# ADVRHumanoids/CentroidalPlanner

Hardware: AMD Instinct MI355X
Metric: NLP eval_g+eval_jac_g throughput (rows/sec) at batch*contacts; HBM GB/s vs peak (higher is better)
Workload: dtype f64; 1 GPU; 4-contact Ground env, batch=1,048,576 (north-star target); contacts=4, environment=ground, batch_per_gpu=1048576, batch_total=1048576, outputs=g + jac (IFOPT CSR values), per-shard residual norms, parallelism=instance-sharded x1, launch=hip-graph, 10 steps per replay

## Files before the change

centroidalplanner_amd/_abi.py:

```python
from __future__ import annotations

import ctypes
import os
from ctypes import POINTER, c_char_p, c_double, c_int32, c_int64, c_size_t, c_uint8, c_void_p

MAX_CONTACTS = 32
ABI_VERSION = 1

ENV_NONE = 0
ENV_GROUND = 1
ENV_SUPERQUADRIC = 2
ENV_MIXED = 3

OK = 0
ERR_INVALID_ARGUMENT = 1
ERR_OUT_OF_RANGE = 2
ERR_RUNTIME = 3
ERR_HIP = 4
ERR_UNSUPPORTED = 5

INF = 1.0e20

EVAL_JAC_FOLDED = 1
EVAL_SOA = 2
# ... 105 lines not shown
    _fields_ = [
        ("d_wrench", c_void_p),
        ("d_com_ref", c_void_p),
        ("d_p_ref", c_void_p),
        ("d_F_ref", c_void_p),
    ]


class DerivativeReport(ctypes.Structure):

    _fields_ = [
        ("n_checked", c_int64),
        ("n_flagged", c_int64),
        ("max_rel_error", c_double),
        ("worst_instance", c_int64),
        ("worst_row", c_int32),
        ("worst_col", c_int32),
        ("worst_exact", c_double),
        ("worst_approx", c_double),
    ]


HESSIAN_EXACT = 0
HESSIAN_LIMITED_MEMORY = 1
HESSIAN_FD = 2
HESSIAN_ANALYTIC = 3

TERM_SCALED = 0
TERM_IPOPT = 1
SOLVE_DIVERGING = 5
SOLVE_TIME_LIMIT = 6

_DESC_P = POINTER(ProblemDesc)
_DP = POINTER(c_double)
_IP = POINTER(c_int32)
SIGNATURES = {
    "cpl_abi_version": (c_int32, []),
    "cpl_desc_sizeof": (c_size_t, []),
    "cpl_last_error": (c_char_p, []),
    "cpl_status_string": (c_char_p, [c_int32]),
    "cpl_desc_init": (c_int32, [_DESC_P, c_int32, c_int32, c_double]),
    "cpl_desc_set_contact_names": (c_int32, [_DESC_P, POINTER(c_char_p), c_int32]),
    "cpl_desc_set_mu": (c_int32, [_DESC_P, c_double]),
    "cpl_desc_set_superquadric": (c_int32, [_DESC_P, _DP, _DP, _DP]),
    "cpl_desc_set_bounds": (c_int32, [_DESC_P, c_int32, c_int32, _DP, _DP]),
    "cpl_dims": (c_int32, [_DESC_P, _IP, _IP, _IP]),
    "cpl_structure": (c_int32, [_DESC_P, _IP, _IP, _IP]),
    "cpl_bounds": (c_int32, [_DESC_P, _DP, _DP, _DP, _DP]),
    "cpl_eval_batch": (
        c_int32,
        [_DESC_P, c_int64, c_void_p, c_void_p, c_void_p, c_void_p, c_void_p, c_void_p, c_void_p, c_void_p],
    ),
    "cpl_set_tuning": (c_int32, [c_int32, c_int32, c_int32, c_int32, c_int32]),
    "cpl_residual_norms": (c_int32, [_DESC_P, c_int64, c_void_p, c_void_p, c_void_p]),
    "cpl_eval_batch_norms": (
        c_int32,
        [_DESC_P, c_int64, c_void_p, c_void_p, c_void_p, c_void_p, c_void_p, c_void_p, c_void_p, c_void_p, c_void_p],
    ),
    "cpl_time_eval_batch": (
        c_int32,
        [_DESC_P, c_int64, c_void_p, c_void_p, c_void_p, c_void_p, c_void_p, c_void_p, c_void_p, c_void_p,
         c_void_p, c_int32, _DP],
    ),
    "cpl_eval_batch_ex": (
        c_int32,
        [_DESC_P, c_int64, c_void_p, c_void_p, c_void_p, c_void_p, c_void_p, c_void_p, c_void_p, c_void_p, c_int32,
         c_void_p],
    ),
    "cpl_instance_data_sizeof": (c_size_t, []),
    "cpl_eval_batch_inst": (
        c_int32,
        [_DESC_P, c_int64, c_void_p, c_void_p, c_void_p, POINTER(InstanceDataC), c_void_p, c_void_p, c_void_p, c_void_p,
         c_void_p, c_int32, c_void_p],
    ),
    "cpl_jac_fold_info": (c_int32, [_DESC_P, _IP, _IP, _IP, _IP, _DP]),
    "cpl_time_eval_batch_ex": (
        c_int32,
        [_DESC_P, c_int64, c_void_p, c_void_p, c_void_p, c_void_p, c_void_p, c_void_p, c_void_p, c_void_p,
         c_int32, c_void_p, c_int32, _DP],
    ),
    "cpl_eval_batch_host": (
        c_int32,
        [_DESC_P, c_int64, c_void_p, c_void_p, c_void_p, c_void_p, c_void_p, c_void_p, c_void_p, c_void_p, c_int32],
    ),
    "cpl_derivative_test": (
        c_int32,
        [_DESC_P, c_int64, c_void_p, c_void_p, c_void_p, c_double, c_double, c_void_p, POINTER(DerivativeReport),
         c_void_p],
    ),
    "cpl_kkt_workspace_doubles": (c_int64, [c_int32, c_int32]),
    "cpl_lagrangian_hessian": (c_int32, [_DESC_P, c_int64, c_void_p, c_void_p, c_void_p, c_void_p, c_int32, c_void_p,
                                         c_void_p]),
    "cpl_lagrangian_hessian_ex": (c_int32, [_DESC_P, c_int64, c_void_p, c_void_p, c_void_p, c_void_p, c_void_p, c_int32,
                                            c_void_p, c_void_p]),
    "cpl_eval_lagrangian_grad": (
        c_int32,
        [_DESC_P, c_int64, c_void_p, c_void_p, c_void_p, c_void_p, c_void_p, c_void_p, c_void_p, c_int32, c_void_p,
         c_void_p, c_void_p],
    ),
    "cpl_lagrangian_grad": (
        c_int32,
        [c_int64, c_int32, c_int32, c_int32, c_void_p, c_void_p, c_void_p, c_void_p, c_void_p, c_void_p, c_int32,
         c_void_p, c_void_p],
    ),
    "cpl_kkt_qd_solve": (c_int32, [c_int64, c_int32, c_int32] + [c_void_p] * 12),
    "cpl_kkt_solve": (
# ... 120 lines not shown
```

centroidalplanner_amd/csrc/cpl_kernels.hip:

```cpp
#include <hip/hip_runtime.h>

#include <cmath>
#include <cstdlib>
#include <cstring>
#include <map>
#include <mutex>
#include <string>
#include <tuple>
#include <vector>

#include "cpl_accept.hpp"
#include "cpl_engine.hpp"
#include "cpl_kkt_block.hpp"
#include "cpl_kkt_wave.hpp"
#include "cpl_layout.hpp"
#include "cpl_wave.hpp"
#include "cpl_status.hpp"

namespace cpl {

constexpr int TILE = 64;
constexpr int CHUNK = 16;
constexpr int SROW = CHUNK + 2;

struct KParams {
  int32_t N, n, m, nnz;
  int32_t env_kind;
  int32_t has_env;
  int32_t x_aligned16;
  int32_t pad0;
  int8_t map_order[CPL_MAX_CONTACTS];
  double mass_default;
  double gravity[3];
  double wrench[6];
  double mu;
  double ground_z;
  double C[3], R[3], P[3];
  double EJ[3];
  double Ka[3];
  double Kb[3];
  double Rm2[3];
  double Rp2[3];
  double Psq[3], Pm1[3], P2[3], P2m2[3], P2m3[3];
  double F_thr[CPL_MAX_CONTACTS];
  double W_com, com_ref[3];
  double W_p[CPL_MAX_CONTACTS], W_F[CPL_MAX_CONTACTS];
  double p_ref[CPL_MAX_CONTACTS][3], F_ref[CPL_MAX_CONTACTS][3];
  int32_t T, logT;
  int32_t S;
  int32_t cost_seg;
  int32_t offG, offJ, offD, offL, offI;
  int32_t LR;
  int32_t offX1, offMB, offTB;
  int32_t want_g, want_j, want_f, want_grad;
  int32_t want_norms;
  int32_t contact_rows;
  int32_t sq_ladder;
  int32_t grid_cap;
  int32_t want_lgrad, y_repeat;
  const int32_t* col_ptr;
  const int32_t* csc_k;
  const int32_t* csc_row;
  const double* ly;
  const uint8_t* lg_active;
  int32_t offC;
  int32_t fold, jbase, cstride;
  int32_t soa;
  int32_t jdirect;
  int32_t offA;
  int32_t offRB, offCS, offST;
  const double* sc_df;
  const double* sc_dc;
  const int32_t* sc_row;
  const uint8_t* gate;
};
static_assert(sizeof(KParams) < 4096, "kernel parameters must fit the kernarg segment");

constexpr int CPL_MAX_ROWS = 6 + 6 * CPL_MAX_CONTACTS;
enum { AX_C, AX_R, AX_P, AX_EJ, AX_KA, AX_KB, AX_RM2, AX_RP2, AX_PSQ, AX_PM1, AX_P2, AX_P2M2, AX_P2M3, AX_N };
struct CTab {
  int32_t map_order[CPL_MAX_CONTACTS];
  double F_thr[CPL_MAX_CONTACTS];
  double ax[AX_N][3];
  uint8_t cone[CPL_MAX_ROWS];
};
__shared__ CTab s_ct;

__device__ __forceinline__ void load_ctab(const KParams& K) {
  const int t = threadIdx.x;
  if (t < CPL_MAX_CONTACTS) {
    s_ct.map_order[t] = K.map_order[t];
    s_ct.F_thr[t] = K.F_thr[t];
  }
  if (t < 3 * AX_N) {
    const int f = t / 3, a = t - 3 * (t / 3);
    double v;
    switch (f) {
      case AX_C: v = K.C[a]; break;
      case AX_R: v = K.R[a]; break;
      case AX_P: v = K.P[a]; break;
      case AX_EJ: v = K.EJ[a]; break;
      case AX_KA: v = K.Ka[a]; break;
      case AX_KB: v = K.Kb[a]; break;
      case AX_RM2: v = K.Rm2[a]; break;
      case AX_RP2: v = K.Rp2[a]; break;
      case AX_PSQ: v = K.Psq[a]; break;
      case AX_PM1: v = K.Pm1[a]; break;
      case AX_P2: v = K.P2[a]; break;
      case AX_P2M2: v = K.P2m2[a]; break;
      default: v = K.P2m3[a]; break;
    }
    s_ct.ax[f][a] = v;
  }
  for (int r = t; r < K.m; r += blockDim.x)
    s_ct.cone[r] = r >= 6 && ((r - 6) % K.contact_rows) >= K.contact_rows - 2;
}

__device__ __forceinline__ double row_violation(double g, bool cone) {
  if (g != g) return INFINITY;
  if (cone) return g > 0.0 ? g : 0.0;
  return fabs(g);
}

struct NormAcc {
  double vmax = 0.0, vsum = 0.0;
  int r = 0, rstep = 0;
  __device__ void init(int tid, int nthreads, int m) {
// ... 1282 lines not shown
        for (int e = tid; e < valid * n; e += WG) {
          const int r = e / n;
          grad_out[rowb[r] * n + (e - r * n)] = Dt[e];
        }
    } else if (K.soa) {
      if (K.want_g) copy_out_soa<WG, NT>(g_out + b0, batch, Gt, m, valid, tid);
      if (K.want_j) copy_out_soa<WG, NT>(jac_out + b0, batch, Jt, nnz, valid, tid);
      if (K.want_grad) copy_out_soa<WG, NT>(grad_out + b0, batch, Dt, n, valid, tid);
    } else {
      if (K.want_g) copy_out<WG, NT>(g_out + b0 * m, Gt, valid * m, tid);
      if (K.want_j && !JD) copy_out<WG, NT>(jac_out + b0 * nnz, Jt, valid * nnz, tid);
      if (K.want_grad) copy_out<WG, NT>(grad_out + b0 * n, Dt, valid * n, tid);
    }
  }
}
using TileKernT = void (*)(const KParams, int64_t, const double*, const double*, const uint8_t*, const int32_t*,
                           const int32_t*, double*, double*, double*, double*, double*);


typedef __attribute__((address_space(3))) void lds_void_t;
typedef __attribute__((address_space(1))) void glb_void_t;


__device__ __forceinline__ void dma_tile(double* dst, const double* src, int count, int lane) {
  const int pieces = (count + 127) >> 7;
  for (int p = 0; p < pieces; ++p) {
    const int e = p * 128 + lane * 2;
    if (e + 1 < count) __builtin_amdgcn_global_load_lds((glb_void_t*)(src + e), (lds_void_t*)(dst + p * 128), 16, 0, 0);
  }
}

template <int CT, bool NT>
__device__ __forceinline__ void copy_out_ct(double* __restrict__ dst, const double* __restrict__ src, int count,
                                            int tid) {
  if ((reinterpret_cast<uintptr_t>(dst) & 15) == 0) {
    const int pairs = count >> 1;
    const double2* s2 = reinterpret_cast<const double2*>(src);
    double2* d2 = reinterpret_cast<double2*>(dst);
    for (int e = tid; e < pairs; e += CT) {
      const double2 v = s2[e];
      if (NT) {
        __builtin_nontemporal_store(v.x, &d2[e].x);
        __builtin_nontemporal_store(v.y, &d2[e].y);
      } else {
        d2[e] = v;
      }
    }
    if ((count & 1) && tid == 0) dst[count - 1] = src[count - 1];
  } else {
    for (int e = tid; e < count; e += CT) dst[e] = src[e];
  }
}

template <int ENVK, int NCW, bool NT, bool SC = false>
__global__ __launch_bounds__(64 * (NCW + 1)) void cpl_eval_pipe_kernel(const KParams K, int64_t batch,
                                                                        const double* __restrict__ x,
                                                                        const double* __restrict__ mass,
                                                                        const uint8_t* __restrict__ env_tag,
                                                                        double* __restrict__ g_out,
                                                                        double* __restrict__ jac_out,
                                                                        double* __restrict__ f_out,
                                                                        double* __restrict__ grad_out,
                                                                        double* __restrict__ norms_ws) {
  constexpr int CT = 64 * NCW;
  constexpr bool HAS_SQ = ENVK == CPL_ENV_SUPERQUADRIC || ENVK == CPL_ENV_MIXED;
  extern __shared__ __align__(16) double smem[];
  if (K.gate && *K.gate == 0) return;
  load_ctab(K);
  int* s_colp = reinterpret_cast<int*>(smem + K.offC);
  int* s_csck = s_colp + K.n + 1;
  int* s_cscr = s_csck + K.nnz;
  if (K.want_lgrad) {
    for (int i = threadIdx.x; i <= K.n; i += blockDim.x) s_colp[i] = K.col_ptr[i];
    for (int i = threadIdx.x; i < K.nnz; i += blockDim.x) {
      s_csck[i] = K.csc_k[i];
      s_cscr[i] = K.csc_row[i];
    }
  }
  __syncthreads();
  const int tid = threadIdx.x;
  const int lane = tid & 63;
  const bool loader = (tid >> 6) == NCW;
  const int T = K.T;
  const int n = K.n, m = K.m, nnz = K.nnz, N = K.N;
  const int64_t ntiles = (batch + T - 1) / T;
  auto XB = [&](int bi) { return smem + (bi ? K.offX1 : 0); };
  auto MB = [&](int bi) { return smem + K.offMB + (bi ? T : 0); };
  auto TB = [&](int bi) { return reinterpret_cast<int*>(smem + K.offTB) + (bi ? T : 0); };
  double* Gt = smem + K.offG;
  double* Jt = smem + K.offJ;
  double* Dt = smem + K.offD;
  double* L = smem + K.offL;
  int* lists = reinterpret_cast<int*>(smem + K.offI);

  int64_t t = blockIdx.x;
  if (t >= ntiles) return;
  double mass_def = K.mass_default;
  asm volatile("" : "+v"(mass_def));
  NormAcc acc;
  acc.init(tid, CT, m);

  double st_mass = 0.0, st_tail = 0.0;
  int st_tag = 0;
  auto stage = [&](int64_t tt, int bi) {
    const int64_t b0s = tt * T;
    const int vs = (int)((batch - b0s) < T ? (batch - b0s) : T);
    const int count = vs * n;
    dma_tile(XB(bi), x + b0s * n, count, lane);
    if ((count & 1) && lane == 0) st_tail = x[b0s * n + count - 1];
    if (lane < vs) {
      st_mass = mass ? mass[b0s + lane] : mass_def;
      if (ENVK == CPL_ENV_MIXED) st_tag = env_tag[b0s + lane];
    }
  };
  auto finish_stage = [&](int64_t tt, int bi) {
    asm volatile("s_waitcnt vmcnt(0)" ::: "memory");
    const int64_t b0s = tt * T;
    const int vs = (int)((batch - b0s) < T ? (batch - b0s) : T);
    const int count = vs * n;
    if ((count & 1) && lane == 0) XB(bi)[count - 1] = st_tail;
    if (lane < vs) {
      MB(bi)[lane] = st_mass;
      if (ENVK == CPL_ENV_MIXED) TB(bi)[lane] = st_tag;
    }
  };

  if (loader) {
    __builtin_amdgcn_s_setprio(3);
    stage(t, 0);
    finish_stage(t, 0);
    lds_barrier();
    int cur = 0;
    for (; t < ntiles; t += gridDim.x) {
      const int64_t tn = t + gridDim.x;
      if (tn < ntiles) stage(tn, cur ^ 1);
      if (ENVK == CPL_ENV_MIXED) lds_barrier();
      if (HAS_SQ) lds_barrier();
      lds_barrier();
      if (tn < ntiles) finish_stage(tn, cur ^ 1);
      lds_barrier();
      cur ^= 1;
    }
  } else {
  lds_barrier();
  int cur = 0;
  for (; t < ntiles; t += gridDim.x) {
    const int64_t b0 = t * T;
    const int valid = (int)((batch - b0) < T ? (batch - b0) : T);
    const double* X = XB(cur);
    if (ENVK == CPL_ENV_MIXED) {
      if (tid < 64) {
        const bool is_sq = tid < valid && TB(cur)[tid] == CPL_ENV_SUPERQUADRIC;
        const unsigned long long msk = __ballot(is_sq);
        if (tid < valid) {
          const int before = __popcll(msk & ((1ull << tid) - 1ull));
          if (is_sq) lists[before] = tid;
          else lists[64 + tid - before] = tid;
        }
        if (tid == 0) lists[128] = __popcll(msk);
      }
      lds_barrier();
    }
    const int n_sq = ENVK == CPL_ENV_SUPERQUADRIC ? valid : (ENVK == CPL_ENV_MIXED ? lists[128] : 0);
    const int n_gr = valid - n_sq;
    const bool wgj = K.want_g || K.want_j;

    const int r_ax = (HAS_SQ && wgj) ? 3 * N * n_sq : 0;
    const int r_gr = (ENVK != CPL_ENV_SUPERQUADRIC && wgj) ? N * n_gr : 0;
    const int r_st = wgj ? 4 * valid : 0;
    const int r_co = K.cost_seg >= 0 ? valid : 0;
    const int items1 = r_ax + r_gr + r_st + r_co;
    const int per_axis = N * n_sq;
    for (int it = tid; it < items1; it += CT) {
      int e = it;
      if (HAS_SQ && e < r_ax) {
        const int a = e / per_axis, kj = e - a * per_axis;
        const int k = kj / n_sq, j = kj - k * n_sq;
        const int r = ENVK == CPL_ENV_MIXED ? lists[j] : j;
        sq_axis_item<ENVK == CPL_ENV_MIXED>(K, X + r * n, k, a, L + r * K.LR + k * SQ_L, Gt + r * m);
        continue;
      }
      e -= r_ax;
      if (e < r_gr) {
        const int j = e % n_gr, k = e / n_gr;
        const int r = ENVK == CPL_ENV_MIXED ? lists[64 + j] : j;
        if (!HAS_SQ && K.lg_active && !K.lg_active[(b0 + r) / K.y_repeat]) continue;
        contact_item<ENVK == CPL_ENV_NONE ? CPL_ENV_NONE : CPL_ENV_GROUND>(K, X + r * n, CPL_ENV_GROUND, k,
// ... 831 lines not shown
              std::memcmp(cache.P, d->sq_P, sizeof(cache.P)) == 0)) {
    for (int a = 0; a < 3; ++a) {
      const double R = d->sq_R[a], P = d->sq_P[a];
      cache.R[a] = R; cache.P[a] = P;
      cache.EJ[a] = P / std::pow(R, P);
      cache.Ka[a] = P * std::pow(R, -P);
      cache.Kb[a] = (P * P) * std::pow(R, P * -2.0);
      cache.Rm2[a] = std::pow(R, -(P * 2.0));
      cache.Rp2[a] = std::pow(R, P * 2.0);
    }
    cache.valid = true;
  }
  for (int a = 0; a < 3; ++a) {
    const double C = d->sq_C[a], R = d->sq_R[a], P = d->sq_P[a];
    K.C[a] = C; K.R[a] = R; K.P[a] = P;
    if (sq) {
      K.EJ[a] = cache.EJ[a]; K.Ka[a] = cache.Ka[a]; K.Kb[a] = cache.Kb[a];
      K.Rm2[a] = cache.Rm2[a]; K.Rp2[a] = cache.Rp2[a];
    }
    K.Psq[a] = P * P;
    K.Pm1[a] = P - 1.0;
    K.P2[a] = P * 2.0;
    K.P2m2[a] = P * 2.0 - 2.0;
    K.P2m3[a] = P * 2.0 - 3.0;
  }
  K.sq_ladder = 1;
  for (int a = 0; a < 3; ++a) {
    const double P = d->sq_P[a];
    if (!(P >= 2.0 && P <= 64.0 && P == std::floor(P))) K.sq_ladder = 0;
  }
  for (int i = 0; i < CPL_MAX_CONTACTS; ++i) {
    K.F_thr[i] = d->F_thr[i];
    K.W_p[i] = d->W_p[i];
    K.W_F[i] = d->W_F[i];
    for (int j = 0; j < 3; ++j) { K.p_ref[i][j] = d->p_ref[i][j]; K.F_ref[i][j] = d->F_ref[i][j]; }
  }
  K.W_com = d->W_com;
  for (int j = 0; j < 3; ++j) K.com_ref[j] = d->com_ref[j];
  K.fold = FOLD_NONE;
  K.jbase = D.statics_nnz;
  K.cstride = D.contact_nnz;
  K.soa = 0;
}

static size_t eval_lds_bytes(int n) { return sizeof(double) * (size_t)(TILE * n + 2 * TILE * SROW); }

enum { VAR_AUTO = 0, VAR_ROWSTAGE = 1, VAR_PIPE = 2, VAR_TILE = 3, VAR_TILE_JD = 4, VAR_ENTRY = 5, VAR_SPLIT = 6,
       VAR_SPLIT_JD = 7 };
static int g_variant = VAR_AUTO;
static size_t g_lds_budget = 0;
static int g_wg = 256;
static int g_nt = 1;

static size_t tile_budget() { return g_lds_budget ? g_lds_budget : 48 * 1024; }
static size_t pipe_budget() { return g_lds_budget ? g_lds_budget : 48 * 1024; }
static bool use_rowstage() { return g_variant == VAR_ROWSTAGE; }
static bool use_pipe(const KParams& K) {
  if (!K.x_aligned16) return false;
  if (g_variant == VAR_PIPE) return true;
  return g_variant == VAR_AUTO && (K.env_kind == CPL_ENV_NONE || K.env_kind == CPL_ENV_GROUND);
}

static int32_t plan_tile(KParams& K, bool g, bool j, bool f, bool grad, int t_max = 64, bool size_without_j = false) {
  const size_t budget = tile_budget();
  K.want_g = g; K.want_j = j; K.want_f = f; K.want_grad = grad;
  const bool sq = K.env_kind == CPL_ENV_SUPERQUADRIC || K.env_kind == CPL_ENV_MIXED;
  K.LR = K.N * SQ_L + 1;
  const size_t per = sizeof(double) * (size_t)(K.n + (g ? K.m : 0) + (j && !K.jdirect ? K.nnz : 0) +
                                               (grad ? K.n : 0) + (sq ? K.LR : 0) + (j && K.jdirect ? 6 : 0));
  const size_t per_t = size_without_j ? per - sizeof(double) * (size_t)(j && !K.jdirect ? K.nnz : 0) : per;
  const size_t fixed = sizeof(double) * 72 + sizeof(CTab);
  int T = 64, logT = 6;
  while (T > t_max) { T >>= 1; --logT; }
  while (T > 2 && (size_t)T * per_t + fixed > budget) { T >>= 1; --logT; }
  if ((size_t)T * per + fixed > 160 * 1024) return fail(CPL_ERR_UNSUPPORTED, "problem too large for one LDS tile");
  K.T = T; K.logT = logT;
  K.cost_seg = (f || grad) ? K.N + 4 : -1;
  K.S = K.N + 4 + ((f || grad) ? 1 : 0);
  K.offG = T * K.n;
  K.offJ = K.offG + (g ? T * K.m : 0);
  K.offD = K.offJ + (j && !K.jdirect ? T * K.nnz : 0);
  K.offL = K.offD + (grad ? T * K.n : 0);
  K.offA = K.offL + (sq ? T * K.LR : 0);
  K.offI = K.offA + (j && K.jdirect ? 6 * T : 0);
  K.offI = (K.offI + 1) & ~1;
  K.offRB = K.offI + 72;
  return CPL_OK;
}

static int32_t plan_pipe(KParams& K, bool g, bool j, bool f, bool grad, size_t extra_fixed = 0) {
  K.want_g = g; K.want_j = j; K.want_f = f; K.want_grad = grad;
  const bool sq = K.env_kind == CPL_ENV_SUPERQUADRIC || K.env_kind == CPL_ENV_MIXED;
  K.LR = K.N * SQ_L + 1;
  const size_t per = sizeof(double) * (size_t)(2 * K.n + 3 + (g ? K.m : 0) + (j ? K.nnz : 0) + (grad ? K.n : 0) +
                                               (sq ? K.LR : 0));
  const size_t fixed = sizeof(double) * (72 + 8) + sizeof(CTab) + extra_fixed;
  int T = 64, logT = 6;
  while (T > 8 && (size_t)T * per + fixed > pipe_budget()) { T >>= 1; --logT; }
  if ((size_t)T * per + fixed > 160 * 1024) return fail(CPL_ERR_UNSUPPORTED, "problem too large for one LDS tile");
  K.T = T; K.logT = logT;
  K.cost_seg = (f || grad) ? K.N + 4 : -1;
  K.S = K.N + 4 + ((f || grad) ? 1 : 0);
  auto up2 = [](int v) { return (v + 1) & ~1; };
  K.offX1 = up2(T * K.n);
  K.offMB = K.offX1 + up2(T * K.n);
  K.offTB = K.offMB + 2 * T;
// ... 106 lines not shown
  hipLaunchKernelGGL(k_kind_write, dim3(nblk), dim3(PART_BLOCK), 0, c.stream, batch, (int)nblk, c.env_tag, kl.blk_sq,
                     kl.idx_gr, kl.idx_sq, kl.counts);
  if ((st = launched(c, "mixed split partition launch"))) return st;
  KParams Kg = K, Ks = K;
  if ((st = plan_entry(Kg, c.g != nullptr, c.jac != nullptr, c.f != nullptr, c.grad != nullptr, true, 40 * 1024)))
    return st;
  Ks.jdirect = (g_variant == VAR_SPLIT_JD && c.jac) ? 1 : 0;
  if ((st = plan_tile(Ks, c.g != nullptr, c.jac != nullptr, c.f != nullptr, c.grad != nullptr))) return st;
  const EntryKernT ek = g_nt ? cpl_eval_entry_kernel<CPL_ENV_GROUND, true> : cpl_eval_entry_kernel<CPL_ENV_GROUND, false>;
  const TileKernT tk = Ks.jdirect ? (g_nt ? cpl_eval_tile_kernel<CPL_ENV_SUPERQUADRIC, 256, true, true, true>
                                          : cpl_eval_tile_kernel<CPL_ENV_SUPERQUADRIC, 256, false, true, true>)
                                  : (g_nt ? cpl_eval_tile_kernel<CPL_ENV_SUPERQUADRIC, 256, true, false, true>
                                          : cpl_eval_tile_kernel<CPL_ENV_SUPERQUADRIC, 256, false, false, true>);
  const size_t lds_g = sizeof(double) * (size_t)Kg.offI;
  const size_t lds_s = sizeof(double) * (size_t)(Ks.offRB + Ks.T);
  if (batch >= (int64_t)1 << 18) Kg.grid_cap = (int32_t)C.cus;
  const unsigned grid_g = persistent_grid((batch + Kg.T - 1) / Kg.T, reinterpret_cast<const void*>(ek), lds_g);
  const unsigned grid_s = (unsigned)((batch + Ks.T - 1) / Ks.T);
  const size_t nparts = (size_t)grid_g + (size_t)grid_s * 4;
  double* ws = nullptr;
  if (c.norms && (st = norm_workspace(C, c.stream, nparts, &ws))) return st;
  if ((st = side_stream(C, c.stream))) return st;
  hipError_t e = hipEventRecord(C.fork, c.stream);
  if (e == hipSuccess) e = hipStreamWaitEvent(C.side, C.fork, 0);
  if (e != hipSuccess) return hip_fail(e, "mixed split fork");
  hipLaunchKernelGGL(tk, dim3(grid_s), dim3(256), lds_s, c.stream, Ks, batch, c.x, c.mass, c.env_tag, kl.idx_sq,
                     kl.counts + 1, c.g, c.jac, c.f, c.grad, ws ? ws + 2 * (size_t)grid_g : nullptr);
  hipLaunchKernelGGL(ek, dim3(grid_g), dim3(256), lds_g, C.side, Kg, batch, c.x, c.mass, kl.idx_gr, kl.counts, c.g,
                     c.jac, c.f, c.grad, ws);
  e = hipGetLastError();
  if (e != hipSuccess) return hip_fail(e, "mixed split launch");
  e = hipEventRecord(C.join, C.side);
  if (e == hipSuccess) e = hipStreamWaitEvent(c.stream, C.join, 0);
  if (e != hipSuccess) return hip_fail(e, "mixed split join");
  return launched(c, "mixed split launch", nparts, ws);
}

static int32_t launch_entry(const EvalCall& c, KParams& K, StreamCtx* C) {
  int32_t st = plan_entry(K, c.g != nullptr, c.jac != nullptr, c.f != nullptr, c.grad != nullptr);
  if (st) return st;
  const size_t lds = sizeof(double) * (size_t)K.offI;
  static const EntryKernT table[2][2] = {
      {cpl_eval_entry_kernel<CPL_ENV_NONE, false>, cpl_eval_entry_kernel<CPL_ENV_NONE, true>},
      {cpl_eval_entry_kernel<CPL_ENV_GROUND, false>, cpl_eval_entry_kernel<CPL_ENV_GROUND, true>}};
  const EntryKernT kern = table[K.env_kind == CPL_ENV_GROUND ? 1 : 0][g_nt ? 1 : 0];
  const unsigned grid = persistent_grid((c.batch + K.T - 1) / K.T, reinterpret_cast<const void*>(kern), lds);
  double* ws = nullptr;
  if (c.norms && (st = norm_workspace(*C, c.stream, grid, &ws))) return st;
  hipLaunchKernelGGL(kern, dim3(grid), dim3(256), lds, c.stream, K, c.batch, c.x, c.mass, nullptr, nullptr, c.g, c.jac,
                     c.f, c.grad, ws);
  return launched(c, "cpl_eval_entry_kernel launch", grid, ws);
}

static int32_t launch_pipe(const EvalCall& c, KParams& K, StreamCtx* C) {
  const LGradArgs* lg = c.lg;
  const int csc_doubles = lg ? (K.n + 1 + 2 * K.nnz + 1) / 2 : 0;
  int32_t st = lg ? plan_pipe(K, false, true, false, true, sizeof(double) * (size_t)csc_doubles)
                  : plan_pipe(K, c.g != nullptr, c.jac != nullptr, c.f != nullptr, c.grad != nullptr);
  if (st) return st;
  K.offC = K.offI + 72;
  if (lg) {
    K.want_lgrad = 1;
    K.y_repeat = lg->y_repeat;
    K.col_ptr = lg->col_ptr;
    K.csc_k = lg->csc_k;
    K.csc_row = lg->csc_row;
    K.ly = lg->y;
    K.lg_active = lg->active;
  }
  const size_t lds = sizeof(double) * (size_t)(K.offC + csc_doubles);
  static const PipeKernT table[4][2] = {
      {cpl_eval_pipe_kernel<CPL_ENV_NONE, 3, false>, cpl_eval_pipe_kernel<CPL_ENV_NONE, 3, true>},
      {cpl_eval_pipe_kernel<CPL_ENV_GROUND, 3, false>, cpl_eval_pipe_kernel<CPL_ENV_GROUND, 3, true>},
      {cpl_eval_pipe_kernel<CPL_ENV_SUPERQUADRIC, 3, false>, cpl_eval_pipe_kernel<CPL_ENV_SUPERQUADRIC, 3, true>},
      {cpl_eval_pipe_kernel<CPL_ENV_MIXED, 3, false>, cpl_eval_pipe_kernel<CPL_ENV_MIXED, 3, true>}};
  static const PipeKernT table_sc[2][2] = {
      {cpl_eval_pipe_kernel<CPL_ENV_NONE, 3, false, true>, cpl_eval_pipe_kernel<CPL_ENV_NONE, 3, true, true>},
      {cpl_eval_pipe_kernel<CPL_ENV_GROUND, 3, false, true>, cpl_eval_pipe_kernel<CPL_ENV_GROUND, 3, true, true>}};
  if (c.sc && K.env_kind != CPL_ENV_NONE && K.env_kind != CPL_ENV_GROUND) return CPL_ERR_UNSUPPORTED;
  if (c.sc) {
    K.sc_df = c.sc->df;
    K.sc_dc = c.sc->dc;
    K.sc_row = c.sc->row;
  }
  const PipeKernT kern =
      c.sc ? table_sc[K.env_kind == CPL_ENV_GROUND ? 1 : 0][g_nt ? 1 : 0] : table[K.env_kind][g_nt ? 1 : 0];
  const unsigned grid = persistent_grid((c.batch + K.T - 1) / K.T, reinterpret_cast<const void*>(kern), lds);
  double* ws = nullptr;
  if (c.norms && (st = norm_workspace(*C, c.stream, grid, &ws))) return st;
  hipLaunchKernelGGL(kern, dim3(grid), dim3(256), lds, c.stream, K, c.batch, c.x, c.mass, c.env_tag, c.g, c.jac, c.f,
                     c.grad, ws);
  return launched(c, "cpl_eval_pipe_kernel launch", grid, ws);
}

static int32_t launch_rowstage(const EvalCall& c, const KParams& K) {
  const size_t lds = eval_lds_bytes(K.n);
  if (lds > 160 * 1024) return fail(CPL_ERR_UNSUPPORTED, "problem too large for one LDS tile");
  const unsigned grid = (unsigned)((c.batch + TILE - 1) / TILE);
  hipLaunchKernelGGL(cpl_eval_kernel, dim3(grid), dim3(TILE), lds, c.stream, K, c.batch, c.x, c.mass, c.env_tag, c.g,
                     c.jac, c.f, c.grad);
  if (int32_t st = launched(c, "cpl_eval_kernel launch")) return st;
  return c.norms && c.finish ? cpl_residual_norms(c.d, c.batch, c.g, c.norms, c.stream) : CPL_OK;
}

static int32_t launch_tile(const EvalCall& c, KParams& K, StreamCtx* C) {
  const bool jd = g_variant == VAR_TILE_JD || (g_variant == VAR_AUTO && K.env_kind == CPL_ENV_MIXED);
  const int wg = g_wg;
  K.jdirect = (jd && c.jac && !K.soa && wg == 256) ? 1 : 0;
  int32_t st = plan_tile(K, c.g != nullptr, c.jac != nullptr, c.f != nullptr, c.grad != nullptr, 64, jd && c.jac);
  if (st) return st;
  const size_t lds = sizeof(double) * (size_t)(K.offRB + K.T);
  const unsigned grid = (unsigned)((c.batch + K.T - 1) / K.T);
  const size_t nparts = (size_t)grid * (wg / 64);
  double* ws = nullptr;
  if (c.norms && (st = norm_workspace(*C, c.stream, nparts, &ws))) return st;
#define CPL_TILE_KERNELS(E) \
  {cpl_eval_tile_kernel<E, 128, false, false>, cpl_eval_tile_kernel<E, 128, true, false>,        \
   cpl_eval_tile_kernel<E, 256, false, false>, cpl_eval_tile_kernel<E, 256, true, false>,        \
   cpl_eval_tile_kernel<E, 256, false, true>, cpl_eval_tile_kernel<E, 256, true, true>}
  static const TileKernT table[4][6] = {CPL_TILE_KERNELS(CPL_ENV_NONE), CPL_TILE_KERNELS(CPL_ENV_GROUND),
                                        CPL_TILE_KERNELS(CPL_ENV_SUPERQUADRIC), CPL_TILE_KERNELS(CPL_ENV_MIXED)};
#undef CPL_TILE_KERNELS
  const TileKernT kern = table[K.env_kind][(K.jdirect ? 4 : (wg == 256 ? 2 : 0)) + (g_nt ? 1 : 0)];
  hipLaunchKernelGGL(kern, dim3(grid), dim3(wg), lds, c.stream, K, c.batch, c.x, c.mass, c.env_tag, nullptr, nullptr,
                     c.g, c.jac, c.f, c.grad, ws);
  return launched(c, "cpl_eval_tile_kernel launch", nparts, ws);
}

static int32_t launch_eval(const EvalCall& c) {
  const cpl_problem_desc* d = c.d;
  int32_t st = validate_desc(d);
  if (st) return st;
  if (c.flags & ~(CPL_EVAL_JAC_FOLDED | CPL_EVAL_SOA)) return fail(CPL_ERR_INVALID_ARGUMENT, "unknown eval flags");
  if (c.batch < 0) return fail(CPL_ERR_INVALID_ARGUMENT, "negative batch");
  if (c.batch == 0) {
    if (c.norms) {
      hipError_t e = hipMemsetAsync(c.norms, 0, 2 * sizeof(double), c.stream);
      if (e != hipSuccess) return hip_fail(e, "hipMemsetAsync norms");
    }
// ... 527 lines not shown
                     dim3((unsigned)batch), dim3(256), 0, (hipStream_t)stream, K, batch, (int)nf, d_x, d_y, d_env_tag,
                     d_active, d_free_idx, d_H);
  hipError_t e = hipGetLastError();
  if (e != hipSuccess) return hip_fail(e, (w + " launch").c_str());
  return CPL_OK;
}

int32_t cpl_lagrangian_hessian(const cpl_problem_desc* d, int64_t batch, const double* d_x, const double* d_y,
                               const uint8_t* d_active, const int32_t* d_free_idx, int32_t nf, double* d_H,
                               void* stream) {
  int32_t st = validate_desc(d);
  if (st) return st;
  if (d->env_kind != CPL_ENV_GROUND && d->env_kind != CPL_ENV_NONE)
    return fail(CPL_ERR_UNSUPPORTED, "cpl_lagrangian_hessian: Ground / no-environment problems only");
  return launch_hessian("cpl_lagrangian_hessian", d, batch, d_x, d_y, nullptr, d_active, d_free_idx, nf, d_H, stream);
}

int32_t cpl_lagrangian_hessian_ex(const cpl_problem_desc* d, int64_t batch, const double* d_x, const double* d_y,
                                  const uint8_t* d_env_tag, const uint8_t* d_active, const int32_t* d_free_idx,
                                  int32_t nf, double* d_H, void* stream) {
  int32_t st = validate_desc(d);
  if (st) return st;
  return launch_hessian("cpl_lagrangian_hessian_ex", d, batch, d_x, d_y, d_env_tag, d_active, d_free_idx, nf, d_H,
                        stream);
}

int32_t cpl_eval_batch_ex(const cpl_problem_desc* d, int64_t batch, const double* d_x, const double* d_mass,
                          const uint8_t* d_env_tag, double* d_g, double* d_jac, double* d_f, double* d_grad,
                          double* d_norms, int32_t flags, void* stream) {
  return launch_eval(EvalCall{d, batch, d_x, d_mass, d_env_tag, d_g, d_jac, d_f, d_grad, d_norms, (hipStream_t)stream, flags});
}

int32_t cpl_eval_batch_norms(const cpl_problem_desc* d, int64_t batch, const double* d_x, const double* d_mass,
                             const uint8_t* d_env_tag, double* d_g, double* d_jac, double* d_f, double* d_grad,
                             double* d_norms, void* stream) {
  if (!d_norms) return fail(CPL_ERR_INVALID_ARGUMENT, "d_norms is required");
  return launch_eval(EvalCall{d, batch, d_x, d_mass, d_env_tag, d_g, d_jac, d_f, d_grad, d_norms, (hipStream_t)stream});
}

int32_t cpl_set_tuning(int32_t kernel_variant, int32_t tile_lds_kb, int32_t wg_threads, int32_t nt_stores,
                       int32_t reserved ) {
  if (reserved != 0) return fail(CPL_ERR_INVALID_ARGUMENT, "the fifth tuning argument is reserved and must be 0");
  if (kernel_variant < VAR_AUTO || kernel_variant > VAR_SPLIT_JD) return fail(CPL_ERR_INVALID_ARGUMENT, "unknown kernel variant");
  if (tile_lds_kb != 0 && (tile_lds_kb < 8 || tile_lds_kb > 160))
    return fail(CPL_ERR_INVALID_ARGUMENT, "LDS budget out of [8, 160] KiB");
  if (wg_threads != 128 && wg_threads != 256) return fail(CPL_ERR_INVALID_ARGUMENT, "workgroup size must be 128 or 256");
  g_variant = kernel_variant;
  g_lds_budget = (size_t)tile_lds_kb * 1024;
  g_wg = wg_threads;
  g_nt = nt_stores ? 1 : 0;
  return CPL_OK;
}

int32_t cpl_residual_norms(const cpl_problem_desc* d, int64_t batch, const double* d_g, double* d_out, void* stream) {
  int32_t st = validate_desc(d);
  if (st) return st;
  if (batch < 0 || !d_out || (batch > 0 && !d_g)) return fail(CPL_ERR_INVALID_ARGUMENT, "bad residual arguments");
  hipStream_t s = (hipStream_t)stream;
  StreamCtx* C = nullptr;
  if ((st = stream_ctx(s, &C))) return st;
  if ((st = ctx_reserve(s, C->rn, RN_GRID, sizeof(double) * 2 * RN_GRID, "residual norms: the per-stream workspace")))
    return st;
  double* ws = static_cast<double*>(C->rn.ptr);
  const Dims D = dims_of(d->n_contacts, d->env_kind);
  const int64_t total = batch * D.m;
  int64_t blocks = (total + RN_BLOCK - 1) / RN_BLOCK;
  if (blocks < 1) blocks = 1;
  if (blocks > RN_GRID) blocks = RN_GRID;
  hipLaunchKernelGGL(cpl_residual_partial, dim3((unsigned)blocks), dim3(RN_BLOCK), 0, s, total, D.m, D.contact_rows,
                     d_g, ws);
  hipError_t e = hipGetLastError();
  if (e != hipSuccess) return hip_fail(e, "cpl_residual_partial launch");
  launch_residual_final((int)blocks, ws, d_out, s);
  e = hipGetLastError();
  if (e != hipSuccess) return hip_fail(e, "cpl_residual_final launch");
  return CPL_OK;
}

int32_t cpl_time_eval_batch(const cpl_problem_desc* d, int64_t batch, const double* d_x, const double* d_mass,
                            const uint8_t* d_env_tag, double* d_g, double* d_jac, double* d_f, double* d_grad,
                            double* d_norms, void* stream, int32_t reps, double* ms_per_launch) {
  return cpl_time_eval_batch_ex(d, batch, d_x, d_mass, d_env_tag, d_g, d_jac, d_f, d_grad, d_norms, 0, stream, reps,
                                ms_per_launch);
}

int32_t cpl_time_eval_batch_ex(const cpl_problem_desc* d, int64_t batch, const double* d_x, const double* d_mass,
                               const uint8_t* d_env_tag, double* d_g, double* d_jac, double* d_f, double* d_grad,
                               double* d_norms, int32_t flags, void* stream, int32_t reps, double* ms_per_launch) {
  if (!ms_per_launch || reps < 1) return fail(CPL_ERR_INVALID_ARGUMENT, "bad timing arguments");
  hipStream_t s = (hipStream_t)stream;
  hipEvent_t e0, e1;
  hipError_t e = hipEventCreate(&e0);
  if (e != hipSuccess) return hip_fail(e, "hipEventCreate");
  e = hipEventCreate(&e1);
  if (e != hipSuccess) { (void)hipEventDestroy(e0); return hip_fail(e, "hipEventCreate"); }
  int32_t st = CPL_OK;
  EvalCall c{d, batch, d_x, d_mass, d_env_tag, d_g, d_jac, d_f, d_grad, d_norms, s, flags};
  c.finish = false;
  (void)hipEventRecord(e0, s);
  for (int32_t r = 0; r < reps && st == CPL_OK; ++r) st = launch_eval(c);
  (void)hipEventRecord(e1, s);
  e = hipEventSynchronize(e1);
  if (st == CPL_OK && e != hipSuccess) st = hip_fail(e, "hipEventSynchronize");
  float ms = 0.0f;
  if (st == CPL_OK) {
    e = hipEventElapsedTime(&ms, e0, e1);
// ... 12 lines not shown
```

include/cpl_mi355x.h:

```cpp
#ifndef CPL_MI355X_H
#define CPL_MI355X_H

#include <stddef.h>
#include <stdint.h>

#ifdef __cplusplus
extern "C" {
#endif

#define CPL_ABI_VERSION 1
#define CPL_MAX_CONTACTS 32

#define CPL_ENV_NONE 0
#define CPL_ENV_GROUND 1
#define CPL_ENV_SUPERQUADRIC 2
#define CPL_ENV_MIXED 3

#define CPL_OK 0
#define CPL_ERR_INVALID_ARGUMENT 1
#define CPL_ERR_OUT_OF_RANGE 2
#define CPL_ERR_RUNTIME 3
#define CPL_ERR_HIP 4
#define CPL_ERR_UNSUPPORTED 5

// ... 43 lines not shown
int32_t cpl_desc_set_bounds(cpl_problem_desc* d, int32_t var, int32_t contact,
                            const double lb[3], const double ub[3]);

int32_t cpl_dims(const cpl_problem_desc* d, int32_t* n, int32_t* m, int32_t* nnz);
int32_t cpl_structure(const cpl_problem_desc* d, int32_t* iRow, int32_t* jCol, int32_t* row_ptr);
int32_t cpl_bounds(const cpl_problem_desc* d, double* x_l, double* x_u, double* g_l, double* g_u);

int32_t cpl_eval_batch(const cpl_problem_desc* d, int64_t batch, const double* d_x,
                       const double* d_mass, const uint8_t* d_env_tag, double* d_g,
                       double* d_jac, double* d_f, double* d_grad, void* stream);

int32_t cpl_residual_norms(const cpl_problem_desc* d, int64_t batch, const double* d_g,
                           double* d_out, void* stream);

int32_t cpl_eval_batch_norms(const cpl_problem_desc* d, int64_t batch, const double* d_x,
                             const double* d_mass, const uint8_t* d_env_tag, double* d_g,
                             double* d_jac, double* d_f, double* d_grad, double* d_norms,
                             void* stream);

#define CPL_EVAL_JAC_FOLDED 1
#define CPL_EVAL_SOA 2

int32_t cpl_eval_batch_ex(const cpl_problem_desc* d, int64_t batch, const double* d_x,
                          const double* d_mass, const uint8_t* d_env_tag, double* d_g,
                          double* d_jac, double* d_f, double* d_grad, double* d_norms,
                          int32_t flags, void* stream);

typedef struct cpl_instance_data {
  const double* d_wrench;
  const double* d_com_ref;
  const double* d_p_ref;
  const double* d_F_ref;
} cpl_instance_data;
size_t cpl_instance_data_sizeof(void);

int32_t cpl_eval_batch_inst(const cpl_problem_desc* d, int64_t batch, const double* d_x, const double* d_mass,
                            const uint8_t* d_env_tag, const cpl_instance_data* inst, double* d_g, double* d_jac,
                            double* d_f, double* d_grad, double* d_norms, int32_t flags, void* stream);

int32_t cpl_jac_fold_info(const cpl_problem_desc* d, int32_t* nnz_folded, int32_t* var_k,
                          int32_t* n_const, int32_t* const_k, double* const_val);

int32_t cpl_time_eval_batch(const cpl_problem_desc* d, int64_t batch, const double* d_x,
                            const double* d_mass, const uint8_t* d_env_tag, double* d_g,
                            double* d_jac, double* d_f, double* d_grad, double* d_norms,
                            void* stream, int32_t reps, double* ms_per_launch);
int32_t cpl_time_eval_batch_ex(const cpl_problem_desc* d, int64_t batch, const double* d_x,
                               const double* d_mass, const uint8_t* d_env_tag, double* d_g,
                               double* d_jac, double* d_f, double* d_grad, double* d_norms,
                               int32_t flags, void* stream, int32_t reps, double* ms_per_launch);

int32_t cpl_set_tuning(int32_t kernel_variant, int32_t tile_lds_kb, int32_t wg_threads, int32_t nt_stores,
                       int32_t reserved);

int32_t cpl_eval_batch_host(const cpl_problem_desc* d, int64_t batch, const double* h_x,
                            const double* h_mass, const uint8_t* h_env_tag, double* h_g,
                            double* h_jac, double* h_f, double* h_grad, double* h_norms,
                            int32_t flags);

typedef struct cpl_derivative_report {
  int64_t n_checked;
  int64_t n_flagged;
  double max_rel_error;
  int64_t worst_instance;
  int32_t worst_row;
  int32_t worst_col;
  double worst_exact, worst_approx;
} cpl_derivative_report;

int32_t cpl_derivative_test(const cpl_problem_desc* d, int64_t batch, const double* d_x,
                            const double* d_mass, const uint8_t* d_env_tag, double perturbation,
                            double tol, int32_t* d_inst_flagged, cpl_derivative_report* report,
                            void* stream);

int64_t cpl_kkt_workspace_doubles(int32_t nw, int32_t m);

int32_t cpl_lagrangian_grad(int64_t batch, int32_t n, int32_t m, int32_t nnz, const int32_t* d_col_ptr,
                            const int32_t* d_csc_k, const int32_t* d_csc_row, const double* d_grad,
                            const double* d_jac, const double* d_y, int32_t y_repeat, double* d_out, void* stream);
int32_t cpl_eval_lagrangian_grad(const cpl_problem_desc* d, int64_t batch, const double* d_x, const double* d_mass,
                                 const uint8_t* d_env_tag, const int32_t* d_col_ptr, const int32_t* d_csc_k,
                                 const int32_t* d_csc_row, const double* d_y, int32_t y_repeat,
                                 const uint8_t* d_active, double* d_out, void* stream);
int32_t cpl_lagrangian_hessian(const cpl_problem_desc* d, int64_t batch, const double* d_x, const double* d_y,
                               const uint8_t* d_active, const int32_t* d_free_idx, int32_t nf, double* d_H,
                               void* stream);
int32_t cpl_lagrangian_hessian_ex(const cpl_problem_desc* d, int64_t batch, const double* d_x, const double* d_y,
                                  const uint8_t* d_env_tag, const uint8_t* d_active, const int32_t* d_free_idx,
                                  int32_t nf, double* d_H, void* stream);
int32_t cpl_kkt_solve(int32_t mode, int64_t batch, int32_t nw, int32_t m, const double* d_M, const double* d_A,
                      const double* d_r1, const double* d_r2, const double* d_mu, const double* d_delta_w_last,
                      const uint8_t* d_active, double* d_dw, double* d_dy, double* d_delta_w, double* d_delta_c,
                      int32_t* d_info, double* d_ws, void* stream);
int32_t cpl_kkt_qd_solve(int64_t batch, int32_t nw, int32_t m, const double* d_W, const double* d_A,
                         const double* d_Dinv, const double* d_r1, const double* d_r2, const uint8_t* d_active,
                         double* d_delta_w_last, double* d_dw, double* d_dy, double* d_delta_w, double* d_ws,
                         void* stream);

int32_t cpl_ipm_trial_point(int64_t batch, int32_t n, int32_t nf, int32_t nw, const int64_t* d_free_idx,
                            const int64_t* d_fixed_idx, const double* d_Xbase, const double* d_w, const double* d_dir,
                            const double* d_alpha, const uint8_t* d_mask, const double* d_w_keep, double* d_wt,
                            double* d_X, void* stream);
int32_t cpl_ipm_judge_take(int64_t batch, int32_t nw, int32_t m, int32_t nf, int32_t nfilt, const int32_t* d_row_slack,
                           const double* d_gl, const uint8_t* d_hasL, const uint8_t* d_hasU, const double* d_wl0,
                           const double* d_wu0, const double* d_wt, const double* d_f_t, const double* d_g_t,
                           const double* d_alpha, const double* d_mu, const double* d_theta_k, const double* d_phi_k,
// ... 149 lines not shown
```

Measured before the change: 78.91 billion rows/s.

## Gate pipe-kernel loader reads into global time windows to separate reads from writes

```diff
diff --git a/centroidalplanner_amd/_abi.py b/centroidalplanner_amd/_abi.py
--- a/centroidalplanner_amd/_abi.py
+++ b/centroidalplanner_amd/_abi.py
@@ -181,6 +181,8 @@
         [_DESC_P, c_int64, c_void_p, c_void_p, c_void_p, c_void_p, c_void_p, c_void_p, c_void_p, c_void_p],
     ),
     "cpl_set_tuning": (c_int32, [c_int32, c_int32, c_int32, c_int32, c_int32]),
+    "cpl_set_read_window": (c_int32, [c_int32, c_int32]),
+    "cpl_read_window_plan": (c_int32, [_DESC_P, c_int64, _IP, _IP]),
     "cpl_residual_norms": (c_int32, [_DESC_P, c_int64, c_void_p, c_void_p, c_void_p]),
     "cpl_eval_batch_norms": (
         c_int32,
diff --git a/centroidalplanner_amd/csrc/cpl_kernels.hip b/centroidalplanner_amd/csrc/cpl_kernels.hip
--- a/centroidalplanner_amd/csrc/cpl_kernels.hip
+++ b/centroidalplanner_amd/csrc/cpl_kernels.hip
@@ -73,6 +73,7 @@
   const double* sc_dc;
   const int32_t* sc_row;
   const uint8_t* gate;
+  int32_t rw_period, rw_open, rw_polls;
 };
 static_assert(sizeof(KParams) < 4096, "kernel parameters must fit the kernarg segment");
 
@@ -1461,7 +1462,18 @@
   }
 }
 
-template <int ENVK, int NCW, bool NT, bool SC = false>
+__device__ __forceinline__ void read_window_wait(uint32_t period, uint32_t open, int polls) {
+  while (polls > 0) {
+    const uint32_t ph = (uint32_t)__builtin_amdgcn_s_memrealtime() % period;
+    if (ph < open) break;
+    int sl = (int)((period - ph) >> 2);
+    sl = sl < 1 ? 1 : sl;
+    polls -= sl;
+    for (; sl > 0; --sl) __builtin_amdgcn_s_sleep(1);
+  }
+}
+
+template <int ENVK, int NCW, bool NT, bool SC = false, bool RW = false>
 __global__ __launch_bounds__(64 * (NCW + 1)) void cpl_eval_pipe_kernel(const KParams K, int64_t batch,
                                                                         const double* __restrict__ x,
                                                                         const double* __restrict__ mass,
@@ -1542,6 +1554,7 @@
     int cur = 0;
     for (; t < ntiles; t += gridDim.x) {
       const int64_t tn = t + gridDim.x;
+      if (RW && tn < ntiles && K.rw_period) read_window_wait((uint32_t)K.rw_period, (uint32_t)K.rw_open, K.rw_polls);
       if (tn < ntiles) stage(tn, cur ^ 1);
       if (ENVK == CPL_ENV_MIXED) lds_barrier();
       if (HAS_SQ) lds_barrier();
@@ -2479,6 +2492,11 @@
 static int g_wg = 256;
 static int g_nt = 1;
 
+static int32_t g_rw_period_ns = 0, g_rw_open_ns = 0;
+constexpr int32_t RW_MAX_PERIOD_NS = 100000;
+constexpr int32_t RW_DEFAULT_PERIOD_NS = 1000, RW_DEFAULT_OPEN_NS = 120;
+constexpr int64_t RW_MIN_BYTES = (int64_t)1 << 29;
+
 static size_t tile_budget() { return g_lds_budget ? g_lds_budget : 48 * 1024; }
 static size_t pipe_budget() { return g_lds_budget ? g_lds_budget : 48 * 1024; }
 static bool use_rowstage() { return g_variant == VAR_ROWSTAGE; }
@@ -2691,6 +2709,22 @@
   return launched(c, "cpl_eval_entry_kernel launch", grid, ws);
 }
 
+static void read_window_policy(const KParams& K, int64_t batch, bool g, bool j, int32_t* period, int32_t* open) {
+  *period = *open = 0;
+  if (K.env_kind != CPL_ENV_NONE && K.env_kind != CPL_ENV_GROUND) return;
+  int32_t pns = g_rw_period_ns, ons = g_rw_open_ns;
+  if (pns < 0) return;
+  if (pns == 0) {
+    const int64_t bytes = batch * (int64_t)sizeof(double) * (K.n + (g ? K.m : 0) + (j ? K.nnz : 0));
+    if (bytes < RW_MIN_BYTES) return;
+    pns = RW_DEFAULT_PERIOD_NS;
+    ons = RW_DEFAULT_OPEN_NS;
+  }
+  *period = pns / 10 > 0 ? pns / 10 : 1;
+  *open = ons / 10 > 0 ? ons / 10 : 1;
+  if (*open > *period) *open = *period;
+}
+
 static int32_t launch_pipe(const EvalCall& c, KParams& K, StreamCtx* C) {
   const LGradArgs* lg = c.lg;
   const int csc_doubles = lg ? (K.n + 1 + 2 * K.nnz + 1) / 2 : 0;
@@ -2722,8 +2756,16 @@
     K.sc_dc = c.sc->dc;
     K.sc_row = c.sc->row;
   }
+  static const PipeKernT table_rw[2][2] = {
+      {cpl_eval_pipe_kernel<CPL_ENV_NONE, 3, false, false, true>, cpl_eval_pipe_kernel<CPL_ENV_NONE, 3, true, false, true>},
+      {cpl_eval_pipe_kernel<CPL_ENV_GROUND, 3, false, false, true>, cpl_eval_pipe_kernel<CPL_ENV_GROUND, 3, true, false, true>}};
+  if (!c.sc && !lg && !c.gate && !K.soa && !K.fold && !c.f && !c.grad)
+    read_window_policy(K, c.batch, c.g != nullptr, c.jac != nullptr, &K.rw_period, &K.rw_open);
+  K.rw_polls = 3 * K.rw_period / 4 + 2;
   const PipeKernT kern =
-      c.sc ? table_sc[K.env_kind == CPL_ENV_GROUND ? 1 : 0][g_nt ? 1 : 0] : table[K.env_kind][g_nt ? 1 : 0];
+      K.rw_period ? table_rw[K.env_kind == CPL_ENV_GROUND ? 1 : 0][g_nt ? 1 : 0]
+      : c.sc      ? table_sc[K.env_kind == CPL_ENV_GROUND ? 1 : 0][g_nt ? 1 : 0]
+                  : table[K.env_kind][g_nt ? 1 : 0];
   const unsigned grid = persistent_grid((c.batch + K.T - 1) / K.T, reinterpret_cast<const void*>(kern), lds);
   double* ws = nullptr;
   if (c.norms && (st = norm_workspace(*C, c.stream, grid, &ws))) return st;
@@ -3357,6 +3399,33 @@
   return CPL_OK;
 }
 
+int32_t cpl_set_read_window(int32_t period_ns, int32_t open_ns) {
+  if (period_ns == -1) {
+    if (open_ns != 0 && open_ns != -1) return fail(CPL_ERR_INVALID_ARGUMENT, "read window: -1 (off) takes no open time");
+  } else {
+    if (period_ns < 0 || open_ns < 0) return fail(CPL_ERR_INVALID_ARGUMENT, "read window: negative time");
+    if (period_ns > RW_MAX_PERIOD_NS) return fail(CPL_ERR_INVALID_ARGUMENT, "read window: period above 100 us");
+    if (open_ns > period_ns) return fail(CPL_ERR_INVALID_ARGUMENT, "read window: open time above the period");
+    if ((period_ns == 0) != (open_ns == 0))
+      return fail(CPL_ERR_INVALID_ARGUMENT, "read window: period and open time are both 0 (default) or both set");
+  }
+  g_rw_period_ns = period_ns;
+  g_rw_open_ns = period_ns > 0 ? open_ns : 0;
+  return CPL_OK;
+}
+
+int32_t cpl_read_window_plan(const cpl_problem_desc* d, int64_t batch, int32_t* period_ticks, int32_t* open_ticks) {
+  int32_t st = validate_desc(d);
+  if (st) return st;
+  if (batch < 0 || !period_ticks || !open_ticks) return fail(CPL_ERR_INVALID_ARGUMENT, "bad read window arguments");
+  KParams K;
+  fill_params(d, K, nullptr);
+  *period_ticks = *open_ticks = 0;
+  if (!use_pipe(K) || use_entry(K, 0)) return CPL_OK;
+  read_window_policy(K, batch, true, true, period_ticks, open_ticks);
+  return CPL_OK;
+}
+
 int32_t cpl_residual_norms(const cpl_problem_desc* d, int64_t batch, const double* d_g, double* d_out, void* stream) {
   int32_t st = validate_desc(d);
   if (st) return st;
diff --git a/include/cpl_mi355x.h b/include/cpl_mi355x.h
--- a/include/cpl_mi355x.h
+++ b/include/cpl_mi355x.h
@@ -119,6 +119,10 @@
 
 int32_t cpl_set_tuning(int32_t kernel_variant, int32_t tile_lds_kb, int32_t wg_threads, int32_t nt_stores,
                        int32_t reserved);
+
+int32_t cpl_set_read_window(int32_t period_ns, int32_t open_ns);
+int32_t cpl_read_window_plan(const cpl_problem_desc* d, int64_t batch, int32_t* period_ticks,
+                             int32_t* open_ticks);
 
 int32_t cpl_eval_batch_host(const cpl_problem_desc* d, int64_t batch, const double* h_x,
                             const double* h_mass, const uint8_t* h_env_tag, double* h_g,
```

Result: faster. 80.13 billion rows/s (median of 6 runs) (+1.5%).
